# rosielab/emojivoice

Measured on NVIDIA B200. Metric: audio_seconds_per_second, higher is better.
Workload: dtype bf16

## Files before the change

### emojivoice_b200/_lib.py

```python
from __future__ import annotations

import ctypes as C
import os

import torch

_HERE = os.path.dirname(os.path.abspath(__file__))
LIB_PATH = os.environ.get("EV_LIB_PATH") or os.path.join(_HERE, "lib", "libemojivoice_b200.so")

PREC = {"fp32": 0, "float32": 0, torch.float32: 0, "bf16": 1, "bfloat16": 1, torch.bfloat16: 1,
        "tf32x3": 2}


class EvTensor(C.Structure):
    _fields_ = [("name", C.c_char_p), ("data", C.c_void_p), ("ndim", C.c_int32), ("shape", C.c_int64 * 4)]


class EvMatchaCfg(C.Structure):
    _fields_ = [(n, C.c_int32) for n in (
        "n_vocab", "n_spks", "spk_emb_dim", "n_feats", "enc_channels", "enc_filter_channels",
        "enc_filter_channels_dp", "enc_heads", "enc_layers", "enc_kernel", "enc_prenet", "dec_channels", "dec_heads",
        "dec_head_dim", "dec_mid_blocks")] + [("mel_mean", C.c_float), ("mel_std", C.c_float)]


# ... 34 lines not shown
    "ev_align_workspace_bytes": (_SZ, [_P, _I, _I, _I]),
    "ev_align": (_I, [_P, _P, _P, _P, _P, _I, _I, _I, _P, _P, _P, _P, _SZ, _P]),
    "ev_decode_workspace_bytes": (_SZ, [_P, _I, _I, _I]),
    "ev_decode": (_I, [_P, _P, _P, _P, _P, _I, _I, _I, _F, _I, _P, _P, _P, _SZ, _P]),
    "ev_vocode_workspace_bytes": (_SZ, [_P, _I, _I]),
    "ev_vocode": (_I, [_P, _P, _I, _I, _I, _P, _P, _SZ, _P]),
    "ev_vocode_ragged": (_I, [_P, _P, _P, _I, _I, _I, _P, _P, _SZ, _P]),
    "ev_denoise_workspace_bytes": (_SZ, [_P, _I, _I]),
    "ev_denoiser_init": (_I, [_P, _P, _P, _SZ, _P]),
    "ev_denoise": (_I, [_P, _P, _I, _I, _F, _P, _P, _SZ, _P]),
    "ev_maximum_path_workspace_bytes": (_SZ, [_P, _I, _I, _I]),
    "ev_maximum_path": (_I, [_P, _P, _P, _P, _I, _I, _I, _F, _P, _P, _SZ, _P]),
    "ev_estimator_workspace_bytes": (_SZ, [_P, _I, _I]),
    "ev_estimator": (_I, [_P, _P, _P, _P, _P, _P, _I, _I, _I, _P, _P, _SZ, _P]),
    "ev_train_forward_workspace_bytes": (_SZ, [_P, _I, _I, _I, _I]),
    "ev_train_forward": (_I, [_P, _P, _P, _P, _P, _P, _P, _P, _P, _P, _I, _P, _I, _I, _I, _F, _I, _I, _P, _P, _P, _SZ, _P]),
    "ev_launch_count": (_I64, [_P, _I]),
    "ev_profile_begin": (_I, [_P]),
    "ev_profile_end": (_I, [_P, C.POINTER(EvKernelStat), _I, C.POINTER(_I)]),
    "ev_test_conv1d": (_I, [_P, _P, _P, _P, _I, _I, _I, _I, _I, _I, _I, _I, _I, _I, _P, _P]),
    "ev_test_attention": (_I, [_P, _P, _P, _I, _I, _I, _I, _I, _P, _P]),
    "ev_test_encoder_attention": (_I, [_P, _P, _P, _I, _I, _I, _I, _P, _I, C.POINTER(_F), _P]),
    "ev_test_encoder_attention_hd": (_I, [_P, _P, _P, _I, _I, _I, _I, _I, _P, _I, C.POINTER(_F), _P]),
    "ev_test_ff_block": (_I, [_P] * 11 + [_I, _I, _I, _I, _P, _I, C.POINTER(_F), _P]),
    "ev_test_tf_tail": (_I, [_P] * 14 + [_I, _I, _I, _I, _P, _I, C.POINTER(_F), _P]),
    "ev_test_resnet_block": (_I, [_P, C.POINTER(EvTensor), _I, _P, _P, _I, _I, _I, _I, _I, _P, _P, _P, _I, C.POINTER(_F), _P]),
    "ev_test_resblock": (_I, [_P, C.POINTER(EvTensor), _I, _I, _I, _P, _P, _I, _I, _I, _F, _F, _I, _I, _P, _I, _I, _I, _I,
                              _P, _P, _P, _P, _P]),
    "ev_test_conv_epilogue": (_I, [_P, C.POINTER(EvConvEpilogueTest), _P]),
    "ev_test_resnet_trace": (_I, [_P, _P, _I]),
    "ev_test_vocoder_margins": (_I, [C.POINTER(EvHifiganCfg), C.POINTER(C.c_int32), C.POINTER(C.c_int32), C.POINTER(C.c_int32)]),
    "ev_test_euler_schedule": (_I, [_I, C.POINTER(_F), C.POINTER(_F)]),
    "ev_test_row_sum": (_I, [_P, _P, _I, _I, _P, _P]),
    "ev_test_conv_trace": (_I, [_P, _P, _I]),
    "ev_test_ff_trace": (_I, [_P, _P, _I]),
}

_lib = None


def lib() -> C.CDLL:
    global _lib
    if _lib is None:
        if not os.path.exists(LIB_PATH):
            raise RuntimeError(
                f"{LIB_PATH} not found: build the CUDA library first (python -m emojivoice_b200.build). "
                "emojivoice_b200 has no CPU or eager-PyTorch fallback.")
        l = C.CDLL(LIB_PATH)
        for name, (res, args) in SIGNATURES.items():
            fn = getattr(l, name)
            fn.restype, fn.argtypes = res, args
        _lib = l
    return _lib


def ptr(t):
    return None if t is None else C.c_void_p(t.data_ptr())


def stream_ptr():
    return C.c_void_p(torch.cuda.current_stream().cuda_stream)


class Context:

    def __init__(self, device=None):
# ... 113 lines not shown
```

### emojivoice_b200/csrc/api.cu

```cuda
#include <algorithm>
#include <cstdlib>
#include <cstring>

#include "ctx.cuh"

using namespace ev;

namespace ev {
bool pdl_enabled() {
  static const bool on = []() { const char* v = getenv("EV_PDL"); return !(v && atoi(v) == 0); }();
  return on;
}
}

namespace {
thread_local std::string g_create_error;
cudaStream_t as_stream(void* s) { return reinterpret_cast<cudaStream_t>(s); }
}

extern "C" int ev_version(void) { return 100; }

extern "C" const char* ev_last_error(const ev_ctx* ctx) { return ctx ? ctx->err.c_str() : g_create_error.c_str(); }

extern "C" int ev_create(ev_ctx** out, int device) {
// ... 658 lines not shown
  return EV_OK;
}

extern "C" int ev_test_resnet_trace(ev_ctx* ctx, uint64_t* out_host, int n) {
  if (!ctx || !out_host || n <= 0) return EV_ERR_INVALID;
  EV_CUDA(ctx, cudaSetDevice(ctx->device));
  EV_CUDA(ctx, cudaDeviceSynchronize());
  EV_CUDA(ctx, resnet_tc_read_trace(reinterpret_cast<unsigned long long*>(out_host), n));
  return EV_OK;
}

extern "C" int ev_test_conv_trace(ev_ctx* ctx, uint64_t* out_host, int n) {
  if (!ctx || !out_host || n <= 0) return EV_ERR_INVALID;
  EV_CUDA(ctx, cudaSetDevice(ctx->device));
  EV_CUDA(ctx, cudaDeviceSynchronize());
  EV_CUDA(ctx, conv_tc_read_trace(reinterpret_cast<unsigned long long*>(out_host), n));
  return EV_OK;
}

extern "C" int ev_test_ff_trace(ev_ctx* ctx, uint64_t* out_host, int n) {
  if (!ctx || !out_host || n <= 0) return EV_ERR_INVALID;
  EV_CUDA(ctx, cudaSetDevice(ctx->device));
  EV_CUDA(ctx, cudaDeviceSynchronize());
  EV_CUDA(ctx, ff_tc_read_trace(reinterpret_cast<unsigned long long*>(out_host), n));
  return EV_OK;
}

extern "C" int ev_test_row_sum(ev_ctx* ctx, const float* x, int B, int Tx, float* out, void* stream) {
  if (!ctx || !x || !out) return EV_ERR_INVALID;
  EV_CUDA(ctx, cudaSetDevice(ctx->device));
  EV_CUDA(ctx, row_sum_aten(x, B, Tx, out, as_stream(stream)));
  return EV_OK;
}
```

### emojivoice_b200/csrc/attention_tc.cu

```cuda
#include <cudaTypedefs.h>

#include "conv.cuh"
#include "kernels.cuh"
#include "tc_ptx.cuh"

namespace ev {
using namespace tc;
namespace {

constexpr int BQ = 128, BKV = 64, HD = 64, STAGES = 3;
constexpr int THREADS = 192;
constexpr int Q_BYTES = BQ * HD * 2, KV_BYTES = BKV * HD * 2, P_BYTES = BQ * BKV * 2;
constexpr int SMEM_BYTES = 1024 + Q_BYTES + STAGES * 2 * KV_BYTES + 2 * P_BYTES;
constexpr uint32_t TMEM_COLS = 256;

struct Params {
  int T, H, inner;
  float c1, c2;
  const int* lens; int len_shift;
  bf16* out; long long out_ld, out_bs;
  int skip_padded_queries;
};

__global__ void __launch_bounds__(THREADS, 2) attn_tc_kernel(const __grid_constant__ CUtensorMap tm, const Params p) {
  extern __shared__ uint8_t smem_raw[];
  __shared__ __align__(8) uint64_t q_full, o_full, kv_full[STAGES], kv_empty[STAGES], s_full[2], s_empty[2], p_full[2], p_empty[2];
  __shared__ uint32_t tmem_base_smem;
  const uint32_t base = (smem_u32(smem_raw) + 1023u) & ~1023u;
  const uint32_t q_s = base, kv_s = base + Q_BYTES, p_s = kv_s + STAGES * 2 * KV_BYTES;
  uint8_t* p_gen = smem_raw + (p_s - smem_u32(smem_raw));
  const int warp = threadIdx.x >> 5, lane = threadIdx.x & 31;
  const int b = blockIdx.z, h = blockIdx.y, q0 = blockIdx.x * BQ;
  const int n_kb = (p.T + BKV - 1) / BKV, n_it = 2 * n_kb;

  if (threadIdx.x == 0) {
    asm volatile("prefetch.tensormap [%0];" ::"l"(&tm) : "memory");
    mbar_init(&q_full, 1); mbar_init(&o_full, 1);
    for (int i = 0; i < STAGES; ++i) { mbar_init(&kv_full[i], 1); mbar_init(&kv_empty[i], 1); }
    for (int i = 0; i < 2; ++i) { mbar_init(&s_full[i], 1); mbar_init(&s_empty[i], 4); mbar_init(&p_full[i], 4); mbar_init(&p_empty[i], 1); }
    asm volatile("fence.mbarrier_init.release.cluster;" ::: "memory");
  }
  if (warp == 5) {
    asm volatile("tcgen05.alloc.cta_group::1.sync.aligned.shared::cta.b32 [%0], %1;" ::"r"(smem_u32(&tmem_base_smem)), "r"(TMEM_COLS) : "memory");
    asm volatile("tcgen05.relinquish_alloc_permit.cta_group::1.sync.aligned;" ::: "memory");
  }
  tcgen05_fence_before();
  __syncthreads();
// ... 38 lines not shown
        for (int k = 0; k < BKV / 16; ++k)
          umma_bf16(tmem_base + 128, da + (uint64_t)(2 * k), db + (uint64_t)(k * 128), idesc_o, (j > 0 || k > 0) ? 1u : 0u);
        umma_commit(&kv_empty[st]);
        umma_commit(&p_empty[pb]);
      }
      __syncwarp();
    };
    mbar_wait(&q_full, 0);
    for (int it = 0; it < n_it; ++it) {
      const int st = it % STAGES, sb = it & 1;
      mbar_wait(&kv_full[st], (uint32_t)(it / STAGES) & 1u);
      mbar_wait(&s_empty[sb], ((uint32_t)(it >> 1) & 1u) ^ 1u);
      tcgen05_fence_after();
      const uint32_t k_t = kv_s + (uint32_t)(st * 2 * KV_BYTES);
      const uint64_t dq = make_smem_desc(q_s), dk = make_smem_desc(k_t);
      if (elect_one()) {
#pragma unroll
        for (int k = 0; k < HD / 16; ++k)
          umma_bf16(tmem_base + (uint32_t)(sb * BKV), dq + (uint64_t)(2 * k), dk + (uint64_t)(2 * k), idesc_s, k > 0 ? 1u : 0u);
        umma_commit(&s_full[sb]);
        if (it < n_kb) umma_commit(&kv_empty[st]);
      }
      __syncwarp();
      if (it > n_kb) issue_pv(it - 1);
    }
    issue_pv(n_it - 1);
    if (elect_one()) umma_commit(&o_full);
    __syncwarp();
  } else {
    const int row = warp * 32 + lane, t = q0 + row;
    const int len = p.lens ? __ldg(p.lens + b) : 0x7fffffff;
    const int n_valid = p.lens ? min(p.T, (len + (1 << p.len_shift) - 1) >> p.len_shift) : p.T;
    const uint32_t lane_addr = tmem_base + ((uint32_t)(warp * 32) << 16);
    float m = -INFINITY;
    for (int it = 0; it < n_kb; ++it) {
      const int sb = it & 1;
      mbar_wait(&s_full[sb], (uint32_t)(it >> 1) & 1u);
      tcgen05_fence_after();
#pragma unroll
      for (int half = 0; half < 2; ++half) {
        uint32_t raw[32];
        tmem_ld32(lane_addr + (uint32_t)(sb * BKV + half * 32), raw);
        const int k0 = it * BKV + half * 32, lim_valid = n_valid - k0, lim_in = p.T - k0;
#pragma unroll
        for (int c = 0; c < 32; ++c) {
          const float x = fmaf(__uint_as_float(raw[c]), p.c1, c < lim_valid ? p.c2 : 0.0f);
          m = fmaxf(m, c < lim_in ? x : -INFINITY);
        }
      }
      tcgen05_fence_before();
      __syncwarp();
      if (lane == 0) mbar_arrive(&s_empty[sb]);
    }
    float l = 0.0f;
    for (int j = 0; j < n_kb; ++j) {
      const int it = n_kb + j, sb = it & 1, pb = j & 1;
      mbar_wait(&s_full[sb], (uint32_t)(it >> 1) & 1u);
      mbar_wait(&p_empty[pb], ((uint32_t)(j >> 1) & 1u) ^ 1u);
      tcgen05_fence_after();
      uint8_t* prow = p_gen + pb * P_BYTES + row * 128;
#pragma unroll
      for (int half = 0; half < 2; ++half) {
        uint32_t raw[32];
        tmem_ld32(lane_addr + (uint32_t)(sb * BKV + half * 32), raw);
        const int k0 = j * BKV + half * 32, lim_valid = n_valid - k0, lim_in = p.T - k0;
        uint32_t pk[16];
#pragma unroll
        for (int c = 0; c < 32; c += 2) {
          const float x0 = fmaf(__uint_as_float(raw[c]), p.c1, c < lim_valid ? p.c2 : 0.0f);
          const float x1 = fmaf(__uint_as_float(raw[c + 1]), p.c1, (c + 1) < lim_valid ? p.c2 : 0.0f);
          const float p0 = c < lim_in ? ex2f(x0 - m) : 0.0f;
          const float p1 = (c + 1) < lim_in ? ex2f(x1 - m) : 0.0f;
          l += p0 + p1;
          __nv_bfloat162 v2 = __floats2bfloat162_rn(p0, p1);
          pk[c >> 1] = *reinterpret_cast<uint32_t*>(&v2);
        }
#pragma unroll
        for (int i = 0; i < 4; ++i) {
          const int ch = (half * 4 + i) ^ (row & 7);
          *reinterpret_cast<uint4*>(prow + ch * 16) = make_uint4(pk[4 * i], pk[4 * i + 1], pk[4 * i + 2], pk[4 * i + 3]);
        }
      }
      tcgen05_fence_before();
      fence_proxy_async();
      __syncwarp();
      if (lane == 0) { mbar_arrive(&s_empty[sb]); mbar_arrive(&p_full[pb]); }
    }
    mbar_wait(&o_full, 0);
    tcgen05_fence_after();
    const float inv = 1.0f / l;
    bf16* orow = p.out + b * p.out_bs + (long long)t * p.out_ld + h * HD;
#pragma unroll
    for (int half = 0; half < 2; ++half) {
      uint32_t raw[32];
      tmem_ld32(lane_addr + (uint32_t)(128 + half * 32), raw);
      if (t < p.T) {
#pragma unroll
        for (int i = 0; i < 4; ++i) {
          uint32_t w[4];
#pragma unroll
          for (int e = 0; e < 4; ++e) {
            __nv_bfloat162 v2 = __floats2bfloat162_rn(__uint_as_float(raw[8 * i + 2 * e]) * inv, __uint_as_float(raw[8 * i + 2 * e + 1]) * inv);
            w[e] = *reinterpret_cast<uint32_t*>(&v2);
          }
          *reinterpret_cast<uint4*>(orow + half * 32 + i * 8) = make_uint4(w[0], w[1], w[2], w[3]);
        }
      }
    }
    tcgen05_fence_before();
  }
  __syncthreads();
  if (warp == 5) {
    tcgen05_fence_after();
    asm volatile("tcgen05.dealloc.cta_group::1.sync.aligned.b32 %0, %1;" ::"r"(tmem_base), "r"(TMEM_COLS) : "memory");
  }
}

}

cudaError_t attention_tc(const AttnTcArgs& a, cudaStream_t s, std::string* err) {
  if (a.D != HD || a.inner != a.H * HD) { if (err) *err = "attention_tc: head_dim must be 64"; return cudaErrorInvalidValue; }
  if ((a.ld & 7) || (a.bs & 7) || (reinterpret_cast<uintptr_t>(a.qkv) & 15) || (a.out_ld & 7) || (a.out_bs & 7) ||
      (reinterpret_cast<uintptr_t>(a.out) & 15)) {
    if (err) *err = "attention_tc: tensors must be 16-byte aligned / strided";
    return cudaErrorInvalidValue;
  }
  CUtensorMap tm;
  if (!tc_encode_bf16_map(&tm, a.qkv, (uint64_t)(3 * a.inner), (uint64_t)a.T, (uint64_t)a.B, (uint64_t)a.ld * 2, (uint64_t)a.bs * 2,
                          HD, BKV, 128, err))
    return cudaErrorInvalidValue;
  static DeviceOnce once;
  cudaError_t ce_attr = once.run([&]() { return cudaFuncSetAttribute(attn_tc_kernel, cudaFuncAttributeMaxDynamicSharedMemorySize, SMEM_BYTES); });
  if (ce_attr != cudaSuccess) return ce_attr;
  Params p;
  p.T = a.T; p.H = a.H; p.inner = a.inner;
  p.c1 = a.scale * 1.4426950408889634f; p.c2 = 1.4426950408889634f;
  p.lens = a.lens; p.len_shift = a.len_shift;
  p.out = a.out; p.out_ld = a.out_ld; p.out_bs = a.out_bs;
  p.skip_padded_queries = a.skip_padded_queries;
  dim3 grid(ceil_div(a.T, BQ), a.H, a.B);
  return launch_pdl(attn_tc_kernel, grid, dim3(THREADS), (size_t)SMEM_BYTES, s, tm, p);
}

}
```

### emojivoice_b200/csrc/kernels.cuh

```cuda
#pragma once
#include "common.cuh"

namespace ev {

template <typename OutT>
cudaError_t cf_to_cl(const float* in, int B, int C, int T, OutT* out, long long out_ld, long long out_bs, float scale,
                     RowMask mask, cudaStream_t s);
cudaError_t cl_to_cf(const float* in, long long in_ld, long long in_bs, int B, int C, int T, float* out, float mul,
                     float add, cudaStream_t s);
cudaError_t i64_to_i32(const long long* in, int* out, int n, cudaStream_t s);
cudaError_t upload_floats(float* dst, const float* vals_host, int n, cudaStream_t s);

cudaError_t embed_tokens(const long long* ids, const float* emb, int B, int Tx, int C, int n_vocab, float scale,
                         RowMask mask, float* out, long long out_ld, long long* flags, cudaStream_t s);
cudaError_t embed_speakers(const long long* ids, const float* table, int B, int dim, int n_spks, float* out, long long* flags ,
                           cudaStream_t s);
cudaError_t fill_speaker_channels(const float* spk, int B, int T, int dim, RowMask mask, float* buf, long long ld,
                                  int c0, cudaStream_t s);

struct LnArgs {
  const float* x = nullptr; long long x_ld = 0;
  const float* add = nullptr; long long add_ld = 0;
  const float* gamma = nullptr; const float* beta = nullptr;
  float eps = 1e-5f;
  int pre_relu = 0, post_relu = 0;
  RowMask mask = {nullptr, 0};
  float* out_f32 = nullptr; long long f32_ld = 0;
  void* out_act = nullptr; long long act_ld = 0;
  void* split = nullptr;
  int B = 0, T = 0, C = 0;
};
template <typename ActT> cudaError_t layer_norm_rows(const LnArgs& a, cudaStream_t s);

struct AttnArgs {
  const float* q = nullptr; const float* k = nullptr; const float* v = nullptr;
  long long ld = 0, bs = 0;
  int B = 0, T = 0, H = 0, D = 0;
  float scale = 1.0f;
  const int* lens = nullptr; int len_shift = 0;
  int mode = 0;
  const float* rope_cos = nullptr; const float* rope_sin = nullptr; int rope_dim = 0;
  void* out = nullptr; long long out_ld = 0, out_bs = 0;
  void* split = nullptr;
};
template <typename ActT> cudaError_t attention_rows(const AttnArgs& a, cudaStream_t s);
bool attention_enc_tc_supported(const AttnArgs& a);
cudaError_t attention_enc_tc(const AttnArgs& a, cudaStream_t s);
struct AttnTcArgs {
  const bf16* qkv = nullptr; long long ld = 0, bs = 0;
  int B = 0, T = 0, H = 0, D = 64, inner = 0;
  float scale = 1.0f;
  const int* lens = nullptr; int len_shift = 0;
  bf16* out = nullptr; long long out_ld = 0, out_bs = 0;
  int skip_padded_queries = 0;
};
cudaError_t attention_tc(const AttnTcArgs& a, cudaStream_t s, std::string* err);
cudaError_t rope_tables(float* cos_t, float* sin_t, int T, int rope_dim, float base, cudaStream_t s);

cudaError_t durations(const float* logw, const int* x_lens, int B, int Tx, float length_scale, float* w_ceil,
                      long long* y_lengths, long long* y_max, cudaStream_t s);
cudaError_t row_sum_aten(const float* x, int B, int Tx, float* out, cudaStream_t s);
cudaError_t generate_path(const float* w_ceil, const int* x_lens, const int* y_lens, int B, int Tx, int T_pad,
                          float* attn, int* frame_token, cudaStream_t s);
cudaError_t gather_mu(const float* mu_x_cf, const int* frame_token, const int* y_lens, int B, int C, int Tx, int T_pad,
                      float* mu_y_cf, float* y_mask, cudaStream_t s);

cudaError_t time_sinusoid(const float* t_steps, int n, int dim, float* out, cudaStream_t s);
template <typename ActT>
cudaError_t decoder_pack_input(const float* z_cf, const float* mu_cf, const float* spk, int B, int F, int S, int T,
                               float temperature, RowMask mask, float* x_state, ActT* xin, long long xin_ld, cudaStream_t s);
cudaError_t group_norm_stats(const float* x, int B, int T, int C, int groups, double* partial, int* n_chunks_out,
                             cudaStream_t s);
struct GnApplyArgs {
  const float* x = nullptr;
  const double* partial = nullptr; int n_chunks = 0;
  const float* gamma = nullptr; const float* beta = nullptr; float eps = 1e-5f;
  int B = 0, T = 0, C = 0, groups = 8;
  RowMask mask = {nullptr, 0};
  const float* temb = nullptr;
  long long temb_bs = 0;
  const float* res = nullptr; long long res_ld = 0;
  float* out_f32 = nullptr; long long f32_ld = 0;
  void* out_act = nullptr; long long act_ld = 0;
  const float* ln_gamma = nullptr; const float* ln_beta = nullptr; void* out_ln = nullptr; long long ln_ld = 0;
};
template <typename ActT> cudaError_t group_norm_apply(const GnApplyArgs& a, cudaStream_t s);

cudaError_t conv_post_tanh(const float* x, int B, int L, int C, const float* w , const float* bias, float* wav,
                           const int* lens, int hop, cudaStream_t s);
// ... 3 lines not shown
```

### emojivoice_b200/csrc/resnet_tc.cu

```cuda
#include <cuda.h>
#include <cudaTypedefs.h>

#include <algorithm>
#include <cstdlib>

#include "conv.cuh"
#include "tc_ptx.cuh"

namespace ev {
using namespace tc;
namespace {

constexpr int RN_C = 256;
constexpr int RN_EPI_WARPS = 16;
constexpr int RN_ROLE_WARPS = 4;
constexpr int RN_THREADS = 32 * (RN_ROLE_WARPS + RN_EPI_WARPS);
constexpr int RN_EPI_THREADS = 32 * RN_EPI_WARPS;
constexpr int RN_W_TILE = 128 * 128;
constexpr int RN_MAX_W_SLOTS = 8;
constexpr int RN_X1_SLOTS = 3, RN_X3_SLOTS = 2;
constexpr int RN_STAGE_WARP = 4096;
constexpr int RN_STAGE = RN_EPI_WARPS * RN_STAGE_WARP;
constexpr int RN_ACT_PITCH = 80;
constexpr int RN_MAX_CLUSTER = 8;
// ... 20 lines not shown
};

__device__ unsigned long long g_rn_trace[32];
#define RN_TR(i) do { if (p.trace && blockIdx.x == 0 && lane == 0) g_rn_trace[(i)] = (unsigned long long)clock64(); } while (0)

__device__ __forceinline__ uint32_t rd_hi(uint32_t sbo, uint32_t layout) { return ((sbo >> 4) & 0x3FFFu) | (1u << 14) | (layout << 29); }
__device__ __forceinline__ uint32_t rd_lo(uint32_t saddr) { return ((saddr & 0x3FFFFu) >> 4) | (1u << 16); }
__device__ __forceinline__ uint64_t rd_join(uint32_t hi, uint32_t lo) { return ((uint64_t)hi << 32) | lo; }

static __device__ __noinline__ void rn_wait_timeout(int line) {
  printf("emojivoice_b200: resnet_tc mbarrier wait at line %d timed out (block %d thread %d)\n", line, blockIdx.x, threadIdx.x);
  __trap();
}
__device__ __forceinline__ void rn_wait_at(uint64_t* bar, uint32_t parity, int line) {
  const uint32_t addr = smem_u32(bar);
  uint32_t spins = 0;
  while (true) {
    uint32_t ok;
    asm volatile(
        "{\n\t.reg .pred p;\n\t"
        "mbarrier.try_wait.parity.shared::cta.b64 p, [%1], %2;\n\t"
        "selp.u32 %0, 1, 0, p;\n\t}"
        : "=r"(ok)
        : "r"(addr), "r"(parity)
        : "memory");
    if (ok) break;
    if (++spins > (1u << 26)) rn_wait_timeout(line);
  }
}
#define RN_WAIT(bar, parity) rn_wait_at((bar), (parity), __LINE__)

__device__ __forceinline__ void epi_bar() { asm volatile("bar.sync 1, %0;" ::"n"(RN_EPI_THREADS) : "memory"); }

__device__ __forceinline__ float mish_add(float x, float add) {
  const float n = ex2f(fminf(x * 1.4426950408889634f, 28.853900817779268f));
  const float d = fmaf(n, n + 2.0f, 2.0f);
  float r;
  asm("rcp.approx.ftz.f32 %0, %1;" : "=f"(r) : "f"(d));
  return fmaf(x, fmaf(-2.0f, r, 1.0f), add);
}
__device__ __forceinline__ uint32_t pack_bf16(float lo, float hi) {
  __nv_bfloat162 v = __floats2bfloat162_rn(lo, hi);
  return *reinterpret_cast<uint32_t*>(&v);
}
__device__ __forceinline__ uint32_t map_to_cta(uint32_t local_saddr, uint32_t rank) {
  uint32_t r;
  asm volatile("mapa.shared::cluster.u32 %0, %1, %2;" : "=r"(r) : "r"(local_saddr), "r"(rank));
  return r;
}
__device__ __forceinline__ void st_async_f32(uint32_t remote_addr, float v, uint32_t remote_bar) {
  asm volatile("st.async.weak.shared::cluster.mbarrier::complete_tx::bytes.b32 [%0], %1, [%2];" ::"r"(remote_addr), "r"(__float_as_uint(v)), "r"(remote_bar) : "memory");
}
__device__ __forceinline__ void cluster_sync_all() {
  asm volatile("barrier.cluster.arrive.release.aligned;\n\tbarrier.cluster.wait.acquire.aligned;" ::: "memory");
}
__global__ void __launch_bounds__(RN_THREADS, 1)
resnet_tc_kernel(const __grid_constant__ RnMaps maps, const __grid_constant__ RnParams p) {
  extern __shared__ uint8_t smem_raw[];
  __shared__ __align__(8) uint64_t x1_full[RN_X1_SLOTS], x1_empty[RN_X1_SLOTS], x3_full[RN_X3_SLOTS], x3_empty[RN_X3_SLOTS];
  __shared__ __align__(8) uint64_t w_full[RN_MAX_W_SLOTS], w_empty[RN_MAX_W_SLOTS];
  __shared__ __align__(8) uint64_t acc_full, plane_ready[2], tm_ready[2], res_full[2], xch_bar[2];
  __shared__ __align__(8) uint64_t qkv_ready, qkv_full[2], qkv_drained;
  __shared__ uint32_t tmem_base_smem;

  const uint32_t base = (smem_u32(smem_raw) + 1023u) & ~1023u;
  uint8_t* base_gen = smem_raw + (base - smem_u32(smem_raw));
  const uint32_t w_s = base, a_s = base + (uint32_t)(p.w_slots * RN_W_TILE);
  uint8_t* a_gen = base_gen + p.w_slots * RN_W_TILE;
  uint8_t* stage_gen = a_gen + (p.a_bytes - RN_STAGE);
  float* cst = reinterpret_cast<float*>(a_gen + p.a_bytes);
  float *c_scale = cst, *c_shift = cst + RN_C, *c_extra = cst + 2 * RN_C, *c_bias = cst + 3 * RN_C, *c_lng = cst + 4 * RN_C, *c_lnb = cst + 5 * RN_C;
  float* rowsum = cst + 6 * RN_C;
// ... 275 lines not shown
      for (int it = 0; it < 4; ++it) {
        const int rr = rsub + it * 8, r = m * 128 + q * 32 + rr, t = m0 - 1 + r;
        if (r >= 1 && r <= R - 2 && t < p.T) *reinterpret_cast<uint4*>(dst + (long long)t * ld + ch * 8) = *reinterpret_cast<const uint4*>(src + rr * RN_ACT_PITCH);
      }
      __syncwarp();
    };

    RN_WAIT(&acc_full, 0);
    tcgen05_fence_after();
    if (ew == 0) RN_TR(2);
    stats_pass(0u);
    exchange(0);
    if (ew == 0) RN_TR(3);
    fold_consts(0, p.g1, p.b1, full ? p.temb + b * p.temb_bs : nullptr, full ? p.bias2 : nullptr);
    if (ew == 0) RN_TR(13);
#pragma unroll 1
    for (int h = 0; h < 2; ++h) {
      const int cb = 4 * h + slot;
      if (ew == 0 && h == 1) RN_TR(14);
#pragma unroll 1
      for (int m = 0; m < p.mb; ++m) {
        const int r = m * 128 + rl, t = m0 - 1 + r;
        const bool valid = t >= 0 && t < p.T && (t << p.len_shift) < len_b;
        uint32_t pk[16];
        if (__any_sync(0xffffffffu, valid)) {
          uint32_t raw[32];
          tmem_ld32(lane_addr + (uint32_t)(m * RN_C + cb * 32), raw);
          if (ew == 0 && h == 0 && m == 0) RN_TR(16);
#pragma unroll
          for (int j = 0; j < 32; j += 4) {
            const int c = cb * 32 + j;
            const float4 sc = *reinterpret_cast<const float4*>(c_scale + c), sh = *reinterpret_cast<const float4*>(c_shift + c);
            const float4 ex = *reinterpret_cast<const float4*>(c_extra + c);
            const float v0 = mish_add(fmaf(__uint_as_float(raw[j]), sc.x, sh.x), ex.x);
            const float v1 = mish_add(fmaf(__uint_as_float(raw[j + 1]), sc.y, sh.y), ex.y);
            const float v2 = mish_add(fmaf(__uint_as_float(raw[j + 2]), sc.z, sh.z), ex.z);
            const float v3 = mish_add(fmaf(__uint_as_float(raw[j + 3]), sc.w, sh.w), ex.w);
            pk[j >> 1] = valid ? pack_bf16(v0, v1) : 0u;
            pk[(j >> 1) + 1] = valid ? pack_bf16(v2, v3) : 0u;
          }
        } else {
#pragma unroll
          for (int j = 0; j < 16; ++j) pk[j] = 0u;
        }
        if (ew == 0 && h == 0 && m == 0) { asm volatile("" ::"r"(pk[0]), "r"(pk[15])); RN_TR(17); }
        if (full) {
          uint8_t* prow = a_gen + (cb >> 1) * (R * 128) + r * 128;
          const int c0 = 4 * (cb & 1), x7 = r & 7;
#pragma unroll
          for (int i = 0; i < 4; ++i)
            *reinterpret_cast<uint4*>(prow + (((c0 + i) ^ x7) << 4)) = make_uint4(pk[4 * i], pk[4 * i + 1], pk[4 * i + 2], pk[4 * i + 3]);
          if (p.a_buf && r >= 1 && r <= R - 2 && t < p.T) {
            uint4* dst = reinterpret_cast<uint4*>(p.a_buf + b * p.a_bs + (long long)t * p.a_ld + cb * 32);
#pragma unroll
            for (int i = 0; i < 4; ++i) dst[i] = make_uint4(pk[4 * i], pk[4 * i + 1], pk[4 * i + 2], pk[4 * i + 3]);
          }
        } else {
          store_bf16_block(pk, p.a_buf + b * p.a_bs + cb * 32, p.a_ld, m);
        }
      }
      if (ew == 0 && h == 0) RN_TR(18);
      if (full) {
        tcgen05_fence_before();
        fence_proxy_async();
        __syncwarp();
        if (lane == 0) mbar_arrive(&plane_ready[h]);
      }
    }
    if (ew == 0) RN_TR(4);
    if (full) {
      RN_WAIT(&acc_full, 1);
      tcgen05_fence_after();
      if (ew == 0) RN_TR(8);
      stats_pass(acc2_col);
      exchange(1);
      if (ew == 0) RN_TR(5);
      fold_consts(1, p.g2, p.b2, p.bias_r, nullptr);
#pragma unroll 1
      for (int h = 0; h < 2; ++h) {
        const int cb = 4 * h + slot;
#pragma unroll 1
        for (int m = 0; m < vmb; ++m) {
          uint32_t raw[32];
          const uint32_t taddr = lane_addr + acc2_col + (uint32_t)(m * RN_C + cb * 32);
          const int t = m0 - 1 + m * 128 + rl;
          const bool valid = t >= 0 && t < p.T && (t << p.len_shift) < len_b;
          if (__any_sync(0xffffffffu, valid)) {
            tmem_ld32(taddr, raw);
#pragma unroll
            for (int j = 0; j < 32; j += 4) {
              const int c = cb * 32 + j;
              const float4 sc = *reinterpret_cast<const float4*>(c_scale + c), sh = *reinterpret_cast<const float4*>(c_shift + c);
              const float4 ex = *reinterpret_cast<const float4*>(c_extra + c);
              const float v0 = mish_add(fmaf(__uint_as_float(raw[j]), sc.x, sh.x), ex.x);
              const float v1 = mish_add(fmaf(__uint_as_float(raw[j + 1]), sc.y, sh.y), ex.y);
              const float v2 = mish_add(fmaf(__uint_as_float(raw[j + 2]), sc.z, sh.z), ex.z);
              const float v3 = mish_add(fmaf(__uint_as_float(raw[j + 3]), sc.w, sh.w), ex.w);
              raw[j] = __float_as_uint(valid ? v0 : ex.x); raw[j + 1] = __float_as_uint(valid ? v1 : ex.y);
              raw[j + 2] = __float_as_uint(valid ? v2 : ex.z); raw[j + 3] = __float_as_uint(valid ? v3 : ex.w);
            }
          } else {
#pragma unroll
            for (int j = 0; j < 32; j += 4) {
              const float4 ex = *reinterpret_cast<const float4*>(c_extra + cb * 32 + j);
              raw[j] = __float_as_uint(ex.x); raw[j + 1] = __float_as_uint(ex.y); raw[j + 2] = __float_as_uint(ex.z); raw[j + 3] = __float_as_uint(ex.w);
            }
          }
          tmem_st32(taddr, raw);
        }
        tmem_st_wait();
        tcgen05_fence_before();
        __syncwarp();
        if (lane == 0) mbar_arrive(&tm_ready[h]);
      }
      if (ew == 0) RN_TR(9);

      const int sub = lane >> 3, cl = lane & 7;
      float ls[2] = {0.0f, 0.0f}, lq[2] = {0.0f, 0.0f};
#pragma unroll 1
      for (int h = 0; h < 2; ++h) {
        const int cb = 4 * h + slot;
        RN_WAIT(&res_full[h], 0);
        tcgen05_fence_after();
        if (ew == 0 && h == 0) RN_TR(11);
#pragma unroll 1
        for (int m = 0; m < vmb; ++m) {
          uint32_t raw[32];
          tmem_ld32(lane_addr + acc2_col + (uint32_t)(m * RN_C + cb * 32), raw);
          float s = 0.0f, qq = 0.0f;
          if (p.xr_cf) {
            const int r = m * 128 + rl, t = m0 - 1 + r;
            const bool own = r >= 1 && r <= R - 2 && t < p.T;
// ... 281 lines not shown
```

### emojivoice_b200/csrc/tc_ptx.cuh

```cuda
#pragma once
#include <cuda.h>

#include "common.cuh"

namespace ev {
namespace tc {

__device__ __forceinline__ uint32_t smem_u32(const void* p) { return (uint32_t)__cvta_generic_to_shared(p); }

__device__ __forceinline__ void mbar_init(uint64_t* bar, uint32_t count) {
  asm volatile("mbarrier.init.shared::cta.b64 [%0], %1;" ::"r"(smem_u32(bar)), "r"(count));
}
__device__ __forceinline__ void mbar_expect_tx(uint64_t* bar, uint32_t bytes) {
  asm volatile("mbarrier.arrive.expect_tx.shared::cta.b64 _, [%0], %1;" ::"r"(smem_u32(bar)), "r"(bytes) : "memory");
}
__device__ __forceinline__ void mbar_arrive(uint64_t* bar) {
  asm volatile("mbarrier.arrive.shared::cta.b64 _, [%0];" ::"r"(smem_u32(bar)) : "memory");
}
static __device__ __noinline__ void mbar_timeout_trap() {
  printf("emojivoice_b200: mbarrier wait timed out (block %d,%d,%d thread %d)\n", blockIdx.x, blockIdx.y, blockIdx.z, threadIdx.x);
  __trap();
}
__device__ __forceinline__ void mbar_wait(uint64_t* bar, uint32_t parity) {
  const uint32_t addr = smem_u32(bar);
// ... 70 lines not shown
      : "memory");
}
__device__ __forceinline__ void tmem_st_wait() { asm volatile("tcgen05.wait::st.sync.aligned;" ::: "memory"); }

__device__ __forceinline__ uint64_t make_smem_desc_ex(uint32_t saddr, uint32_t sbo, uint32_t lbo, uint32_t layout) {
  uint64_t d = 0;
  d |= (uint64_t)((saddr & 0x3FFFFu) >> 4);
  d |= (uint64_t)((lbo >> 4) & 0x3FFFu) << 16;
  d |= (uint64_t)((sbo >> 4) & 0x3FFFu) << 32;
  d |= (uint64_t)1 << 46;
  d |= (uint64_t)layout << 61;
  return d;
}
__device__ __forceinline__ uint64_t make_smem_desc(uint32_t saddr) { return make_smem_desc_ex(saddr, 1024, 16, 2); }
__host__ __device__ constexpr uint32_t make_idesc(int m, int n, int a_mn = 0, int b_mn = 0) {
  return (1u << 4) | (1u << 7) | (1u << 10) | ((uint32_t)a_mn << 15) | ((uint32_t)b_mn << 16) |
         ((uint32_t)(n >> 3) << 17) | ((uint32_t)(m >> 4) << 24);
}
__host__ __device__ constexpr uint32_t make_idesc_tf32(int m, int n) {
  return (1u << 4) | (2u << 7) | (2u << 10) | ((uint32_t)(n >> 3) << 17) | ((uint32_t)(m >> 4) << 24);
}
__device__ __forceinline__ void umma_tf32(uint32_t tmem_d, uint64_t desc_a, uint64_t desc_b, uint32_t idesc, uint32_t accumulate) {
  asm volatile(
      "{\n\t.reg .pred p;\n\t"
      "setp.ne.b32 p, %4, 0;\n\t"
      "tcgen05.mma.cta_group::1.kind::tf32 [%0], %1, %2, %3, p;\n\t}"
      ::"r"(tmem_d), "l"(desc_a), "l"(desc_b), "r"(idesc), "r"(accumulate)
      : "memory");
}
__device__ __forceinline__ void mbar_arrive_cnt(uint64_t* bar) { mbar_arrive(bar); }
__device__ __forceinline__ void fence_proxy_async() { asm volatile("fence.proxy.async.shared::cta;" ::: "memory"); }
__device__ __forceinline__ float ex2f(float x) { float y; asm("ex2.approx.ftz.f32 %0, %1;" : "=f"(y) : "f"(x)); return y; }

}
}
```

### include/emojivoice_b200.h

```cpp
#ifndef EMOJIVOICE_B200_H
#define EMOJIVOICE_B200_H

#include <stddef.h>
#include <stdint.h>

#if defined(__GNUC__)
#define EV_API __attribute__((visibility("default")))
#else
#define EV_API
#endif

#ifdef __cplusplus
extern "C" {
#endif

typedef struct ev_ctx ev_ctx;

typedef enum {
  EV_OK = 0,
  EV_ERR_INVALID = -1,
  EV_ERR_CUDA = -2,
  EV_ERR_MISSING = -3,
  EV_ERR_STATE = -4,
  EV_ERR_NO_DEVICE = -5
// ... 106 lines not shown
              int B, int L, int mode, float inv_n, float slope_out, int write_f32, int want_act, const int64_t* lengths,
              int rows_per_frame, int margin, int impl, int precision, const int32_t* schedule, float* sum, float* act,
              int32_t* report, void* stream);
typedef struct {
  int32_t B, C_in, T, C_out, K, stride, pad, dilation, transposed, precision;
  const float* w;
  const float* bias;
  const void* x;
  int64_t x_ld, x_bs;
  const float* res;
  int64_t res_ld, res_bs;
  const float* res2;
  int64_t res2_ld, res2_bs;
  float* out_f32;
  int64_t f32_ld, f32_bs;
  void* out_act;
  int64_t act_ld, act_bs;
  double* gn_sum;
  const int64_t* lengths;
  const float* snake_a;
  const float* snake_invb;
  int32_t gn_groups, len_shift, mask_pre, mask_act, act, f32_is_act;
  float slope, alpha, div;
  int32_t ragged_margin, rows_per_frame;
  const int64_t* ragged_lengths;
  const int32_t* schedule_host;
  int32_t* report_host;
} ev_conv_epilogue_test;
EV_API int ev_test_conv_epilogue(ev_ctx* ctx, const ev_conv_epilogue_test* args, void* stream);
EV_API int ev_test_resnet_trace(ev_ctx* ctx, uint64_t* out_host, int n);
EV_API int ev_test_vocoder_margins(const ev_hifigan_cfg* cfg, int32_t* stage, int32_t* up, int32_t* pre);
EV_API int ev_test_euler_schedule(int n_timesteps, float* t_host, float* dt_host);
EV_API int ev_test_row_sum(ev_ctx* ctx, const float* x, int B, int Tx, float* out, void* stream);
EV_API int ev_test_ff_trace(ev_ctx* ctx, uint64_t* out_host, int n);
EV_API int ev_test_conv_trace(ev_ctx* ctx, uint64_t* out_host, int n);

#ifdef __cplusplus
}
#endif
#endif
```

Measured before the change: 8592.

## Offload part of exp2 to packed FMA polynomial in attention and Mish epilogues

Adds a packed-FMA (float2) polynomial exp2 emulation and uses it for a fraction of the exponentials in the attention softmax and the ResNet Mish epilogue, splitting work between the MUFU unit and the FMA pipes. Attention also gets a fast path for uniformly valid 32-column halves: max is taken on raw scores before scaling, and masking is skipped. The aim is to relieve the special-function-unit bottleneck in the epilogues. It adds polynomial approximation error and more register pressure, plus a test entry point for the new exp2.

```diff
diff --git a/emojivoice_b200/_lib.py b/emojivoice_b200/_lib.py
--- a/emojivoice_b200/_lib.py
+++ b/emojivoice_b200/_lib.py
@@ -90,6 +90,7 @@
     "ev_test_vocoder_margins": (_I, [C.POINTER(EvHifiganCfg), C.POINTER(C.c_int32), C.POINTER(C.c_int32), C.POINTER(C.c_int32)]),
     "ev_test_euler_schedule": (_I, [_I, C.POINTER(_F), C.POINTER(_F)]),
     "ev_test_row_sum": (_I, [_P, _P, _I, _I, _P, _P]),
+    "ev_test_fastmath": (_I, [_I, _P, C.c_int64, _P, _P]),
     "ev_test_conv_trace": (_I, [_P, _P, _I]),
     "ev_test_ff_trace": (_I, [_P, _P, _I]),
 }
diff --git a/emojivoice_b200/csrc/api.cu b/emojivoice_b200/csrc/api.cu
--- a/emojivoice_b200/csrc/api.cu
+++ b/emojivoice_b200/csrc/api.cu
@@ -714,3 +714,8 @@
   EV_CUDA(ctx, row_sum_aten(x, B, Tx, out, as_stream(stream)));
   return EV_OK;
 }
+
+extern "C" int ev_test_fastmath(int kind, const float* x, int64_t n, float* out, void* stream) {
+  if (kind != 0 || !x || !out || n < 0) return EV_ERR_INVALID;
+  return fastmath_exp2(x, (long long)n, out, as_stream(stream)) == cudaSuccess ? EV_OK : EV_ERR_CUDA;
+}
diff --git a/emojivoice_b200/csrc/attention_tc.cu b/emojivoice_b200/csrc/attention_tc.cu
--- a/emojivoice_b200/csrc/attention_tc.cu
+++ b/emojivoice_b200/csrc/attention_tc.cu
@@ -13,6 +13,7 @@
 constexpr int Q_BYTES = BQ * HD * 2, KV_BYTES = BKV * HD * 2, P_BYTES = BQ * BKV * 2;
 constexpr int SMEM_BYTES = 1024 + Q_BYTES + STAGES * 2 * KV_BYTES + 2 * P_BYTES;
 constexpr uint32_t TMEM_COLS = 256;
+constexpr int POLY_PAIRS = 3;
 
 struct Params {
   int T, H, inner;
@@ -117,6 +118,7 @@
     const int len = p.lens ? __ldg(p.lens + b) : 0x7fffffff;
     const int n_valid = p.lens ? min(p.T, (len + (1 << p.len_shift) - 1) >> p.len_shift) : p.T;
     const uint32_t lane_addr = tmem_base + ((uint32_t)(warp * 32) << 16);
+    auto uniform_half = [&](int k0) { return k0 + 32 <= p.T && (k0 + 32 <= n_valid || k0 >= n_valid); };
     float m = -INFINITY;
     for (int it = 0; it < n_kb; ++it) {
       const int sb = it & 1;
@@ -127,10 +129,17 @@
         uint32_t raw[32];
         tmem_ld32(lane_addr + (uint32_t)(sb * BKV + half * 32), raw);
         const int k0 = it * BKV + half * 32, lim_valid = n_valid - k0, lim_in = p.T - k0;
-#pragma unroll
-        for (int c = 0; c < 32; ++c) {
-          const float x = fmaf(__uint_as_float(raw[c]), p.c1, c < lim_valid ? p.c2 : 0.0f);
-          m = fmaxf(m, c < lim_in ? x : -INFINITY);
+        if (uniform_half(k0)) {
+          float s = __uint_as_float(raw[0]);
+#pragma unroll
+          for (int c = 1; c < 32; ++c) s = fmaxf(s, __uint_as_float(raw[c]));
+          m = fmaxf(m, fmaf(s, p.c1, lim_valid > 0 ? p.c2 : 0.0f));
+        } else {
+#pragma unroll
+          for (int c = 0; c < 32; ++c) {
+            const float x = fmaf(__uint_as_float(raw[c]), p.c1, c < lim_valid ? p.c2 : 0.0f);
+            m = fmaxf(m, c < lim_in ? x : -INFINITY);
+          }
         }
       }
       tcgen05_fence_before();
@@ -138,6 +147,7 @@
       if (lane == 0) mbar_arrive(&s_empty[sb]);
     }
     float l = 0.0f;
+    float2 l2 = make_float2(0.0f, 0.0f);
     for (int j = 0; j < n_kb; ++j) {
       const int it = n_kb + j, sb = it & 1, pb = j & 1;
       mbar_wait(&s_full[sb], (uint32_t)(it >> 1) & 1u);
@@ -150,15 +160,28 @@
         tmem_ld32(lane_addr + (uint32_t)(sb * BKV + half * 32), raw);
         const int k0 = j * BKV + half * 32, lim_valid = n_valid - k0, lim_in = p.T - k0;
         uint32_t pk[16];
-#pragma unroll
-        for (int c = 0; c < 32; c += 2) {
-          const float x0 = fmaf(__uint_as_float(raw[c]), p.c1, c < lim_valid ? p.c2 : 0.0f);
-          const float x1 = fmaf(__uint_as_float(raw[c + 1]), p.c1, (c + 1) < lim_valid ? p.c2 : 0.0f);
-          const float p0 = c < lim_in ? ex2f(x0 - m) : 0.0f;
-          const float p1 = (c + 1) < lim_in ? ex2f(x1 - m) : 0.0f;
-          l += p0 + p1;
-          __nv_bfloat162 v2 = __floats2bfloat162_rn(p0, p1);
-          pk[c >> 1] = *reinterpret_cast<uint32_t*>(&v2);
+        if (uniform_half(k0)) {
+          const float o = (lim_valid > 0 ? p.c2 : 0.0f) - m;
+          const float2 c1 = make_float2(p.c1, p.c1), off = make_float2(o, o);
+#pragma unroll
+          for (int c = 0; c < 32; c += 2) {
+            const float2 x = __ffma2_rn(make_float2(__uint_as_float(raw[c]), __uint_as_float(raw[c + 1])), c1, off);
+            const float2 e = ((c >> 1) & 7) < POLY_PAIRS ? exp2_fma2(x) : make_float2(ex2f(x.x), ex2f(x.y));
+            l2 = __fadd2_rn(l2, e);
+            __nv_bfloat162 v2 = __floats2bfloat162_rn(e.x, e.y);
+            pk[c >> 1] = *reinterpret_cast<uint32_t*>(&v2);
+          }
+        } else {
+#pragma unroll
+          for (int c = 0; c < 32; c += 2) {
+            const float x0 = fmaf(__uint_as_float(raw[c]), p.c1, c < lim_valid ? p.c2 : 0.0f);
+            const float x1 = fmaf(__uint_as_float(raw[c + 1]), p.c1, (c + 1) < lim_valid ? p.c2 : 0.0f);
+            const float p0 = c < lim_in ? ex2f(x0 - m) : 0.0f;
+            const float p1 = (c + 1) < lim_in ? ex2f(x1 - m) : 0.0f;
+            l += p0 + p1;
+            __nv_bfloat162 v2 = __floats2bfloat162_rn(p0, p1);
+            pk[c >> 1] = *reinterpret_cast<uint32_t*>(&v2);
+          }
         }
 #pragma unroll
         for (int i = 0; i < 4; ++i) {
@@ -173,7 +196,7 @@
     }
     mbar_wait(&o_full, 0);
     tcgen05_fence_after();
-    const float inv = 1.0f / l;
+    const float inv = 1.0f / (l + (l2.x + l2.y));
     bf16* orow = p.out + b * p.out_bs + (long long)t * p.out_ld + h * HD;
 #pragma unroll
     for (int half = 0; half < 2; ++half) {
@@ -201,6 +224,19 @@
   }
 }
 
+__global__ void exp2_fma2_kernel(const float* __restrict__ x, long long n, float* __restrict__ y) {
+  for (long long i = 2 * ((long long)blockIdx.x * blockDim.x + threadIdx.x); i < n; i += 2LL * gridDim.x * blockDim.x) {
+    const float2 r = exp2_fma2(make_float2(x[i], i + 1 < n ? x[i + 1] : 0.0f));
+    y[i] = r.x;
+    if (i + 1 < n) y[i + 1] = r.y;
+  }
+}
+
+}
+
+cudaError_t fastmath_exp2(const float* x, long long n, float* y, cudaStream_t s) {
+  exp2_fma2_kernel<<<1184, 256, 0, s>>>(x, n, y);
+  return cudaGetLastError();
 }
 
 cudaError_t attention_tc(const AttnTcArgs& a, cudaStream_t s, std::string* err) {
diff --git a/emojivoice_b200/csrc/kernels.cuh b/emojivoice_b200/csrc/kernels.cuh
--- a/emojivoice_b200/csrc/kernels.cuh
+++ b/emojivoice_b200/csrc/kernels.cuh
@@ -55,6 +55,7 @@
   int skip_padded_queries = 0;
 };
 cudaError_t attention_tc(const AttnTcArgs& a, cudaStream_t s, std::string* err);
+cudaError_t fastmath_exp2(const float* x, long long n, float* y, cudaStream_t s);
 cudaError_t rope_tables(float* cos_t, float* sin_t, int T, int rope_dim, float base, cudaStream_t s);
 
 cudaError_t durations(const float* logw, const int* x_lens, int B, int Tx, float length_scale, float* w_ceil,
diff --git a/emojivoice_b200/csrc/resnet_tc.cu b/emojivoice_b200/csrc/resnet_tc.cu
--- a/emojivoice_b200/csrc/resnet_tc.cu
+++ b/emojivoice_b200/csrc/resnet_tc.cu
@@ -76,12 +76,27 @@
 
 __device__ __forceinline__ void epi_bar() { asm volatile("bar.sync 1, %0;" ::"n"(RN_EPI_THREADS) : "memory"); }
 
-__device__ __forceinline__ float mish_add(float x, float add) {
-  const float n = ex2f(fminf(x * 1.4426950408889634f, 28.853900817779268f));
-  const float d = fmaf(n, n + 2.0f, 2.0f);
+__device__ __forceinline__ float rcp_approx(float d) {
   float r;
   asm("rcp.approx.ftz.f32 %0, %1;" : "=f"(r) : "f"(d));
-  return fmaf(x, fmaf(-2.0f, r, 1.0f), add);
+  return r;
+}
+template <bool poly>
+__device__ __forceinline__ float2 mish_add2(float2 raw, float2 sc, float2 sh, float2 add) {
+  const float2 x = __ffma2_rn(raw, sc, sh);
+  float2 z = __fmul2_rn(x, make_float2(1.4426950408889634f, 1.4426950408889634f));
+  z = make_float2(fminf(z.x, 28.853900817779268f), fminf(z.y, 28.853900817779268f));
+  const float2 n = poly ? exp2_fma2(z) : make_float2(ex2f(z.x), ex2f(z.y));
+  const float2 d = __ffma2_rn(n, __fadd2_rn(n, make_float2(2.0f, 2.0f)), make_float2(2.0f, 2.0f));
+  const float2 r = make_float2(rcp_approx(d.x), rcp_approx(d.y));
+  return __ffma2_rn(x, __ffma2_rn(make_float2(-2.0f, -2.0f), r, make_float2(1.0f, 1.0f)), add);
+}
+__device__ __forceinline__ float4 mish_add4(const uint32_t* raw, float4 sc, float4 sh, float4 add) {
+  const float2 a = mish_add2<true>(make_float2(__uint_as_float(raw[0]), __uint_as_float(raw[1])), make_float2(sc.x, sc.y),
+                                   make_float2(sh.x, sh.y), make_float2(add.x, add.y));
+  const float2 b = mish_add2<false>(make_float2(__uint_as_float(raw[2]), __uint_as_float(raw[3])), make_float2(sc.z, sc.w),
+                                    make_float2(sh.z, sh.w), make_float2(add.z, add.w));
+  return make_float4(a.x, a.y, b.x, b.y);
 }
 __device__ __forceinline__ uint32_t pack_bf16(float lo, float hi) {
   __nv_bfloat162 v = __floats2bfloat162_rn(lo, hi);
@@ -423,12 +438,9 @@
             const int c = cb * 32 + j;
             const float4 sc = *reinterpret_cast<const float4*>(c_scale + c), sh = *reinterpret_cast<const float4*>(c_shift + c);
             const float4 ex = *reinterpret_cast<const float4*>(c_extra + c);
-            const float v0 = mish_add(fmaf(__uint_as_float(raw[j]), sc.x, sh.x), ex.x);
-            const float v1 = mish_add(fmaf(__uint_as_float(raw[j + 1]), sc.y, sh.y), ex.y);
-            const float v2 = mish_add(fmaf(__uint_as_float(raw[j + 2]), sc.z, sh.z), ex.z);
-            const float v3 = mish_add(fmaf(__uint_as_float(raw[j + 3]), sc.w, sh.w), ex.w);
-            pk[j >> 1] = valid ? pack_bf16(v0, v1) : 0u;
-            pk[(j >> 1) + 1] = valid ? pack_bf16(v2, v3) : 0u;
+            const float4 v = mish_add4(raw + j, sc, sh, ex);
+            pk[j >> 1] = valid ? pack_bf16(v.x, v.y) : 0u;
+            pk[(j >> 1) + 1] = valid ? pack_bf16(v.z, v.w) : 0u;
           }
         } else {
 #pragma unroll
@@ -483,12 +495,9 @@
               const int c = cb * 32 + j;
               const float4 sc = *reinterpret_cast<const float4*>(c_scale + c), sh = *reinterpret_cast<const float4*>(c_shift + c);
               const float4 ex = *reinterpret_cast<const float4*>(c_extra + c);
-              const float v0 = mish_add(fmaf(__uint_as_float(raw[j]), sc.x, sh.x), ex.x);
-              const float v1 = mish_add(fmaf(__uint_as_float(raw[j + 1]), sc.y, sh.y), ex.y);
-              const float v2 = mish_add(fmaf(__uint_as_float(raw[j + 2]), sc.z, sh.z), ex.z);
-              const float v3 = mish_add(fmaf(__uint_as_float(raw[j + 3]), sc.w, sh.w), ex.w);
-              raw[j] = __float_as_uint(valid ? v0 : ex.x); raw[j + 1] = __float_as_uint(valid ? v1 : ex.y);
-              raw[j + 2] = __float_as_uint(valid ? v2 : ex.z); raw[j + 3] = __float_as_uint(valid ? v3 : ex.w);
+              const float4 v = mish_add4(raw + j, sc, sh, ex);
+              raw[j] = __float_as_uint(valid ? v.x : ex.x); raw[j + 1] = __float_as_uint(valid ? v.y : ex.y);
+              raw[j + 2] = __float_as_uint(valid ? v.z : ex.z); raw[j + 3] = __float_as_uint(valid ? v.w : ex.w);
             }
           } else {
 #pragma unroll
diff --git a/emojivoice_b200/csrc/tc_ptx.cuh b/emojivoice_b200/csrc/tc_ptx.cuh
--- a/emojivoice_b200/csrc/tc_ptx.cuh
+++ b/emojivoice_b200/csrc/tc_ptx.cuh
@@ -126,5 +126,22 @@
 __device__ __forceinline__ void fence_proxy_async() { asm volatile("fence.proxy.async.shared::cta;" ::: "memory"); }
 __device__ __forceinline__ float ex2f(float x) { float y; asm("ex2.approx.ftz.f32 %0, %1;" : "=f"(y) : "f"(x)); return y; }
 
+__device__ __forceinline__ float2 exp2_fma2(float2 x) {
+  const float2 magic = make_float2(12582912.0f, 12582912.0f);
+  const float2 t = __fadd2_rn(x, magic);
+  const float2 r = __fadd2_rn(t, make_float2(-12582912.0f, -12582912.0f));
+  const float2 f = __ffma2_rn(r, make_float2(-1.0f, -1.0f), x);
+  float2 p = __ffma2_rn(f, make_float2(1.53456480e-4f, 1.53456480e-4f), make_float2(1.33998750e-3f, 1.33998750e-3f));
+  p = __ffma2_rn(p, f, make_float2(9.61848907e-3f, 9.61848907e-3f));
+  p = __ffma2_rn(p, f, make_float2(5.55032901e-2f, 5.55032901e-2f));
+  p = __ffma2_rn(p, f, make_float2(2.40226462e-1f, 2.40226462e-1f));
+  p = __ffma2_rn(p, f, make_float2(6.93147182e-1f, 6.93147182e-1f));
+  p = __ffma2_rn(p, f, make_float2(1.0f, 1.0f));
+  const float2 s = make_float2(__uint_as_float((__float_as_uint(t.x) << 23) + 0x3F800000u),
+                               __uint_as_float((__float_as_uint(t.y) << 23) + 0x3F800000u));
+  const float2 y = __fmul2_rn(p, s);
+  return make_float2(x.x < -126.0f ? 0.0f : y.x, x.y < -126.0f ? 0.0f : y.y);
+}
+
 }
 }
diff --git a/include/emojivoice_b200.h b/include/emojivoice_b200.h
--- a/include/emojivoice_b200.h
+++ b/include/emojivoice_b200.h
@@ -162,6 +162,7 @@
 EV_API int ev_test_vocoder_margins(const ev_hifigan_cfg* cfg, int32_t* stage, int32_t* up, int32_t* pre);
 EV_API int ev_test_euler_schedule(int n_timesteps, float* t_host, float* dt_host);
 EV_API int ev_test_row_sum(ev_ctx* ctx, const float* x, int B, int Tx, float* out, void* stream);
+EV_API int ev_test_fastmath(int kind, const float* x, int64_t n, float* out, void* stream);
 EV_API int ev_test_ff_trace(ev_ctx* ctx, uint64_t* out_host, int n);
 EV_API int ev_test_conv_trace(ev_ctx* ctx, uint64_t* out_host, int n);
 
```

Result: no change. 8680, median of 6 (+1.0%).
